# yunjinli/visual-slam

Hardware: AMD Instinct MI355X
Metric: stereo frames/sec, detect+describe (1500 feats) + stereo match, 752x480 (higher is better)
Workload: dtype u8/f32/f64; 1 GPU; synthetic 752x480 stereo, 1500 feats/frame (BASELINE configs[1]); independent streams per GPU (configs[3]); inputs_resident_in_hbm=True, distinct_stereo_pairs_per_gpu=1024, distinct_scenes_per_gpu=64, stereo_frames_per_pass_per_gpu=1024, hip_streams=2, stereo_frames_per_launch=512, num_features=1500, match=threshold 70, ratio 1.2, cross-check

## Files before the change

### visual-slam_amd/csrc/detect.hip

```cpp
#include <type_traits>

#include "vsl_common.h"

#ifndef K1_ROWS
#define K1_ROWS 60
#endif
#ifndef K1_ROWS_SMALL
#define K1_ROWS_SMALL 29
#endif
#define VSL_QUALITY_LEVEL 0.01
#define K1_WLIST 384
#define K1_COLS 60

__device__ __forceinline__ int reflect101(int i, int n) { return i < 0 ? -i : (i >= n ? 2 * n - 2 - i : i); }

struct RowF {
  float rx, ry;
};

struct RowRaw {
  unsigned l, m, r;
};

typedef __amdgpu_buffer_rsrc_t ImgSrd;
__device__ __forceinline__ RowRaw rowload(ImgSrd img, int w, int yr, unsigned xm, unsigned xe, unsigned xp) {
  const int row = yr * w;
  RowRaw o;
  o.l = __builtin_amdgcn_raw_buffer_load_b8(img, (int)xm, row, 0);
  o.m = __builtin_amdgcn_raw_buffer_load_b8(img, (int)xe, row, 0);
  o.r = __builtin_amdgcn_raw_buffer_load_b8(img, (int)xp, row, 0);
  return o;
}

__device__ __forceinline__ RowF rowfilt(RowRaw p, float s, float s2) {
  const float l = (float)p.l, m = (float)p.m, r = (float)p.r;
  RowF o;
  o.rx = r - l;
  float t = s * l;
  t = t + s2 * m;
  t = t + s * r;
  o.ry = t;
  return o;
}

__device__ __forceinline__ float from_lane_below(float v) {
  return __builtin_bit_cast(float, __builtin_amdgcn_update_dpp(0, __builtin_bit_cast(int, v), 0x138, 0xf, 0xf, true));
}
__device__ __forceinline__ float from_lane_above(float v) {
  return __builtin_bit_cast(float, __builtin_amdgcn_update_dpp(0, __builtin_bit_cast(int, v), 0x130, 0xf, 0xf, true));
}

__device__ __forceinline__ double dpp_below_f64(double v) {
  const uint64_t b = __builtin_bit_cast(uint64_t, v);
  const uint32_t lo = (uint32_t)__builtin_amdgcn_update_dpp(0, (int)(uint32_t)b, 0x138, 0xf, 0xf, true);
  const uint32_t hi = (uint32_t)__builtin_amdgcn_update_dpp(0, (int)(uint32_t)(b >> 32), 0x138, 0xf, 0xf, true);
  return __builtin_bit_cast(double, ((uint64_t)hi << 32) | lo);
}

__device__ __forceinline__ double dpp_above_f64(double v) {
  const uint64_t b = __builtin_bit_cast(uint64_t, v);
  const uint32_t lo = (uint32_t)__builtin_amdgcn_update_dpp(0, (int)(uint32_t)b, 0x130, 0xf, 0xf, true);
  const uint32_t hi = (uint32_t)__builtin_amdgcn_update_dpp(0, (int)(uint32_t)(b >> 32), 0x130, 0xf, 0xf, true);
  return __builtin_bit_cast(double, ((uint64_t)hi << 32) | lo);
}

__device__ __forceinline__ float fmax3(float a, float b, float c) {
  float r;
  asm("v_max3_f32 %0, %1, %2, %3" : "=v"(r) : "v"(a), "v"(b), "v"(c));
  return r;
}

__device__ __forceinline__ float fmax2(float a, float b) {
  float r;
  asm("v_max_f32 %0, %1, %2" : "=v"(r) : "v"(a), "v"(b));
  return r;
}

#define K1_SQRT_FLOOR 0x1p-100f
__device__ __forceinline__ float fast_sqrt_rn(float t) {
  const float y = __builtin_amdgcn_rsqf(__builtin_fmaxf(t, K1_SQRT_FLOOR));
  const float r = t * y;
  const float e = __builtin_fmaf(-r, r, t);
  return __builtin_fmaf(e, 0.5f * y, r);
}
__device__ __forceinline__ float sqrt_rn(float t) {
  float r = fast_sqrt_rn(t);
  const bool small = t < K1_SQRT_FLOOR;
  if (__builtin_amdgcn_ballot_w64(small) != 0ull) {
    asm volatile("" ::: "memory");
    const bool rare = small && t > 0.f;
    if (__builtin_amdgcn_ballot_w64(rare) != 0ull) {
      asm volatile("" ::: "memory");
      if (rare) r = sqrtf(t);
    }
  }
  return r;
}

__global__ void sqrt_check_kernel(uint32_t lo, uint32_t hi, unsigned long long* bad) {
  const uint64_t stride = (uint64_t)gridDim.x * blockDim.x;
  unsigned long long n = 0;
  for (uint64_t b = (uint64_t)lo + blockIdx.x * blockDim.x + threadIdx.x; b <= hi; b += stride) {
    const float t = __builtin_bit_cast(float, (uint32_t)b);
    n += __builtin_bit_cast(uint32_t, fast_sqrt_rn(t)) != __builtin_bit_cast(uint32_t, sqrtf(t));
  }
  if (n) atomicAdd(bad, n);
}

__global__ void detect_init_kernel(int32_t* meta, int first, int n) {
  const int i = blockIdx.x * blockDim.x + threadIdx.x;
  if (i < n) {
    meta[(size_t)(first + i) * VSL_META_STRIDE + VSL_META_MAX] = INT32_MIN;
    meta[(size_t)(first + i) * VSL_META_STRIDE + VSL_META_NCAND] = 0;
  }
}

template <bool STORE_RESPONSE, int ROWS>
__global__ __launch_bounds__(256) void min_eig_response_kernel(const uint8_t* __restrict__ images,
                                                               float* __restrict__ response, int32_t* __restrict__ meta,
                                                               uint64_t* __restrict__ cand, size_t cand_cap, int w, int h,
                                                               int first, int wlist_cap, int n_images, int tiles_x, int tiles_y) {
  __shared__ uint64_t list[4][K1_WLIST];
  __shared__ int wave_n[4], wave_max[4], g_base;
  __shared__ double xbuf[4][2][66];
  const int tiles = tiles_x * tiles_y;
  int img_i, tile;
  if (n_images >= 8) {
    const int xcd = blockIdx.x & 7, sl = blockIdx.x >> 3;
    img_i = (sl / tiles) * 8 + xcd;
    tile = sl - (sl / tiles) * tiles;
  } else {
    img_i = blockIdx.x / tiles;
    tile = blockIdx.x - img_i * tiles;
  }
  if (img_i >= n_images) return;
  const int bx = tile % tiles_x, by = tile / tiles_x;
  const int slot = first + img_i;
  const ImgSrd img = __builtin_amdgcn_make_buffer_rsrc((void*)(images + (size_t)slot * w * h), 0, w * h, 0x00020000);
  float* __restrict__ resp = response + (size_t)slot * w * h;
  const int lane = threadIdx.x & 63;
  const int wave = __builtin_amdgcn_readfirstlane(threadIdx.x >> 6);
  const int xs = bx * K1_COLS;
  const int y0 = (by * 4 + wave) * ROWS;
  int n_wave = 0;
  int own_max = INT32_MIN;
  if (y0 < h) {
    const float s = (float)(1.0 / (4.0 * 3.0 * 255.0));
    const float s2 = 2.0f * s;
    const int x = xs - 2 + lane;
    const unsigned xe = (unsigned)reflect101(min(max(x, -1), w), w);
    const unsigned xm = (unsigned)reflect101((int)xe - 1, w), xp = (unsigned)reflect101((int)xe + 1, w);
    const bool own_col = lane >= 2 && lane < 2 + K1_COLS && x < w;
    const bool cand_col = own_col && x >= 1 && x < w - 1;
    const unsigned long long cand_lanes = __builtin_amdgcn_ballot_w64(cand_col);

    struct R3 {
      double xx, xy, yy;
    };
    R3 ra = {0, 0, 0}, rb = ra, bs = ra;
    float va = 0.f, vb = 0.f, hA = 0.f, hB = 0.f, hC = 0.f;
    RowF fA = {0.f, 0.f}, fB = fA, fC = fA;
    int prev_ye = -100, pre_row = -100;
    RowRaw pre = {0u, 0u, 0u};
    float vmax = -3.0e38f;
    const int y_end = min(h, y0 + ROWS);
    auto step = [&](auto steady_tag, auto even_tag, int q, R3& r2, R3& r1, float& v_mid_slot, float& v_dn_slot, float& h_up,
                    float& h_mid, float& h_dn, RowF& f0, RowF& f1, RowF& f2) {
      constexpr bool STEADY = decltype(steady_tag)::value;
      constexpr bool EVEN = decltype(even_tag)::value;
      if (STEADY) {
        f2 = rowfilt(pre, s, s2);
        pre = rowload(img, w, min(q + 2, h - 1), xm, xe, xp);
      } else {
        const int ye = reflect101(min(max(q, -1), h), h);
        if (ye == prev_ye + 1 && ye + 1 < h) {
          if (pre_row != ye + 1) pre = rowload(img, w, ye + 1, xm, xe, xp);
          f2 = rowfilt(pre, s, s2);
        } else {
          f0 = rowfilt(rowload(img, w, reflect101(ye - 1, h), xm, xe, xp), s, s2);
          f1 = rowfilt(rowload(img, w, ye, xm, xe, xp), s, s2);
          f2 = rowfilt(rowload(img, w, reflect101(ye + 1, h), xm, xe, xp), s, s2);
        }
        pre_row = min(ye + 2, h - 1);
        pre = rowload(img, w, pre_row, xm, xe, xp);
        prev_ye = ye;
      }
      const float dx = (f0.rx + f2.rx) * s + f1.rx * s2;
      const float dy = f2.ry - f0.ry;
      const double dxx = (double)(dx * dx), dxy = (double)(dx * dy), dyy = (double)(dy * dy);
      R3 cur;
      {
        xbuf[wave][0][lane + 1] = dxx;
        xbuf[wave][1][lane + 1] = dxy;
        asm volatile("" ::: "memory");
        const double lxx = xbuf[wave][0][lane], uxx = xbuf[wave][0][lane + 2];
        const double lxy = xbuf[wave][1][lane], uxy = xbuf[wave][1][lane + 2];
        asm volatile("" ::: "memory");
        cur.xx = (lxx + dxx) + uxx;
        cur.xy = (lxy + dxy) + uxy;
        cur.yy = (dpp_below_f64(dyy) + dyy) + dpp_above_f64(dyy);
      }
      const int y = q - 1;
      double Axx, Axy, Ayy;
      if (EVEN) {
        bs.xx = r1.xx + cur.xx;
        bs.xy = r1.xy + cur.xy;
        bs.yy = r1.yy + cur.yy;
        Axx = r2.xx + bs.xx;
        Axy = r2.xy + bs.xy;
        Ayy = r2.yy + bs.yy;
      } else {
        Axx = bs.xx + cur.xx;
        Axy = bs.xy + cur.xy;
        Ayy = bs.yy + cur.yy;
      }
      r2 = cur;
      const float X = (float)Axx, b = (float)Axy, Y = (float)Ayy;
      const float xpy = X + Y, d = 0.5f * (X - Y);
      float t = d * d;
      t = t + b * b;
      const float v_dn = __builtin_fmaf(0.5f, xpy, -sqrt_rn(t));
      float h_tmp;
      asm volatile("s_nop 1\n\tv_max_f32_dpp %0, %2, %2 wave_shr:1 row_mask:0xf bank_mask:0xf bound_ctrl:0\n\t"
                   "v_max_f32_dpp %1, %2, %0 wave_shl:1 row_mask:0xf bank_mask:0xf bound_ctrl:0"
                   : "=&v"(h_tmp), "=&v"(h_dn)
                   : "v"(v_dn));
      if (own_col && y >= y0 && y < y_end) {
        if (STORE_RESPONSE) resp[y * w + x] = v_dn;
        vmax = fmax2(vmax, v_dn);
      }
      const float v_mid = v_mid_slot;
      const int yc = q - 2;
      if (yc >= y0 && yc < y_end && yc >= 1 && yc < h - 1) {
        const float m9 = fmax3(h_up, h_mid, h_dn);
        const bool ge0 = v_mid >= m9;
        if ((__builtin_amdgcn_ballot_w64(ge0) & cand_lanes) != 0ull) {
          const bool ge = ge0 && v_mid > 0.f;
          const unsigned long long mask = __builtin_amdgcn_ballot_w64(ge) & cand_lanes;
          if (cand_col && ge) {
            const uint32_t ob = (uint32_t)vsl_float_to_ordered(v_mid) ^ 0x80000000u;
            const uint64_t key = ((uint64_t)ob << 32) | ((uint32_t)yc << 16) | (uint32_t)x;
            const int p = n_wave + (int)__builtin_amdgcn_mbcnt_hi((uint32_t)(mask >> 32),
                                                                  __builtin_amdgcn_mbcnt_lo((uint32_t)mask, 0u));
            if (__builtin_expect(p < wlist_cap, 1)) {
              list[wave][p] = key;
            } else {
              const int g = atomicAdd(&meta[(size_t)slot * VSL_META_STRIDE + VSL_META_NCAND], 1);
              if ((size_t)g < cand_cap) cand[(size_t)slot * cand_cap + g] = key;
            }
          }
          n_wave += __popcll(mask);
        }
      }
      v_dn_slot = v_dn;
    };
    const int q_first = y0 - 2, q_last = y_end + 1;
    typedef std::integral_constant<bool, true> Steady;
    typedef std::integral_constant<bool, false> Generic;
    typedef std::integral_constant<bool, true> Even;
    typedef std::integral_constant<bool, false> Odd;
#define K1_STEP_E0(T, q) step(T{}, Even{}, q, ra, rb, va, vb, hA, hB, hC, fA, fB, fC)
#define K1_STEP_O1(T, q) step(T{}, Odd{}, q, rb, ra, vb, va, hB, hC, hA, fB, fC, fA)
#define K1_STEP_E2(T, q) step(T{}, Even{}, q, ra, rb, va, vb, hC, hA, hB, fC, fA, fB)
#define K1_STEP_O3(T, q) step(T{}, Odd{}, q, rb, ra, vb, va, hA, hB, hC, fA, fB, fC)
#define K1_STEP_E4(T, q) step(T{}, Even{}, q, ra, rb, va, vb, hB, hC, hA, fB, fC, fA)
#define K1_STEP_O5(T, q) step(T{}, Odd{}, q, rb, ra, vb, va, hC, hA, hB, fC, fA, fB)
    constexpr int K1_OPEN = (ROWS + 4) % 6;
    static_assert(K1_OPEN == 3 || K1_OPEN == 4, "opening sequence written for 3 or 4 steps");
#define K1_STRIP(T)                                \
  K1_STEP_E0(Generic, q_first);                    \
  K1_STEP_O1(T, q_first + 1);                      \
  K1_STEP_E2(T, q_first + 2);                      \
  if constexpr (K1_OPEN == 3) {                    \
    for (int q = q_first + 3; q <= q_last; q += 6) { \
      K1_STEP_O3(T, q);                            \
      K1_STEP_E4(T, q + 1);                        \
      K1_STEP_O5(T, q + 2);                        \
      K1_STEP_E0(T, q + 3);                        \
      K1_STEP_O1(T, q + 4);                        \
      K1_STEP_E2(T, q + 5);                        \
    }                                              \
  } else {                                         \
    K1_STEP_O3(T, q_first + 3);                    \
    for (int q = q_first + 4; q <= q_last; q += 6) { \
      K1_STEP_E4(T, q);                            \
      K1_STEP_O5(T, q + 1);                        \
      K1_STEP_E0(T, q + 2);                        \
      K1_STEP_O1(T, q + 3);                        \
      K1_STEP_E2(T, q + 4);                        \
      K1_STEP_O3(T, q + 5);                        \
    }                                              \
  }
    if (q_first >= 1 && q_last + 1 < h) {
      K1_STRIP(Steady)
    } else {
      K1_STRIP(Generic)
    }
#undef K1_STRIP
#undef K1_STEP_E0
#undef K1_STEP_O1
#undef K1_STEP_E2
#undef K1_STEP_O3
#undef K1_STEP_E4
#undef K1_STEP_O5
#pragma unroll
    for (int o = 32; o > 0; o >>= 1) vmax = fmaxf(vmax, __shfl_xor(vmax, o));
    own_max = vsl_float_to_ordered(vmax);
    if (lane == 0) atomicMax(&meta[(size_t)slot * VSL_META_STRIDE + VSL_META_MAX], own_max);
  }
  if (lane == 0) wave_max[wave] = own_max;
  __syncthreads();
  int kept = min(n_wave, wlist_cap);
  {
    const float wg_max = vsl_ordered_to_float(max(max(wave_max[0], wave_max[1]), max(wave_max[2], wave_max[3])));
    if (wg_max > 0.f && kept > 0) {
      const float thr = (float)((double)wg_max * VSL_QUALITY_LEVEL);
      const uint32_t floor_hi = (uint32_t)vsl_float_to_ordered(thr) ^ 0x80000000u;
      const int have = kept;
      kept = 0;
      for (int i0 = 0; i0 < have; i0 += 64) {
        const int i = i0 + lane;
        const uint64_t key = i < have ? list[wave][i] : 0ull;
        const bool keep = i < have && (uint32_t)(key >> 32) > floor_hi;
        const unsigned long long m = __builtin_amdgcn_ballot_w64(keep);
        if (keep) list[wave][kept + (int)__builtin_amdgcn_mbcnt_hi((uint32_t)(m >> 32), __builtin_amdgcn_mbcnt_lo((uint32_t)m, 0u))] = key;
        kept += __popcll(m);
      }
    }
  }
  if (lane == 0) wave_n[wave] = kept;
  __syncthreads();
  const int c0 = wave_n[0], c1 = wave_n[1], c2 = wave_n[2], c3 = wave_n[3];
  const int n = c0 + c1 + c2 + c3;
  if (n == 0) return;
  if (threadIdx.x == 0) g_base = atomicAdd(&meta[(size_t)slot * VSL_META_STRIDE + VSL_META_NCAND], n);
  __syncthreads();
  const int base = g_base + (wave > 0 ? c0 : 0) + (wave > 1 ? c1 : 0) + (wave > 2 ? c2 : 0);
  const int mine = wave_n[wave];
  for (int i = lane; i < mine; i += 64)
    if ((size_t)(base + i) < cand_cap) cand[(size_t)slot * cand_cap + base + i] = list[wave][i];
}

#define SEL_THREADS 1024
#define SEL_CHUNK 8192
#define SEL_BINS 1024
#define SEL_MAX_BLOCKERS 6
static_assert(SEL_THREADS <= 1024 && SEL_MAX_BLOCKERS * 10 <= 64, "blocker packing");

struct SelShared {
  int wave_tot[16];
  int hist[256];
  unsigned long long sel_prefix;
  int sel_k;
  int n_chunk;
};

__device__ __forceinline__ int block_scan(bool p, int* wave_tot, int& total) {
  const int lane = threadIdx.x & 63, wave = __builtin_amdgcn_readfirstlane(threadIdx.x >> 6);
  const unsigned long long m = __ballot(p);
  const int within = (int)__builtin_amdgcn_mbcnt_hi((uint32_t)(m >> 32), __builtin_amdgcn_mbcnt_lo((uint32_t)m, 0u));
  const int mine = __popcll(m);
  __syncthreads();
  if (lane == 0) wave_tot[wave] = mine;
  __syncthreads();
  int x = wave_tot[lane & 15];
  x += __builtin_amdgcn_update_dpp(0, x, 0x111, 0xf, 0xf, true);
  x += __builtin_amdgcn_update_dpp(0, x, 0x112, 0xf, 0xf, true);
  x += __builtin_amdgcn_update_dpp(0, x, 0x114, 0xf, 0xf, true);
  x += __builtin_amdgcn_update_dpp(0, x, 0x118, 0xf, 0xf, true);
  total = __builtin_amdgcn_readlane(x, 15);
  return __builtin_amdgcn_readlane(x, wave) - mine + within;
}

#define SEL_MAX_CELLS 6144
#define SEL_ACC_VALID 0x40u
#define SEL_HEAD_EMPTY 0xFFFFu
#define SEL_KEYS_PADDED (SEL_CHUNK + SEL_CHUNK / 32)
#define SEL_PHYS(i) ((i) + ((i) >> 5))
#define SEL_GRID_BYTES (SEL_MAX_CELLS * 2 * 2)
#define SEL_STAGE_PAD (SEL_CHUNK * 4 - SEL_THREADS * 4 - SEL_GRID_BYTES)
#define SEL_LDS_BYTES (SEL_KEYS_PADDED * 8 + 2048 + SEL_THREADS * 4 * 3 + SEL_GRID_BYTES + SEL_STAGE_PAD)
static_assert(SEL_STAGE_PAD >= 0, "ranking staging array");
static_assert(SEL_LDS_BYTES <= 160 * 1024 - 39344, "selection kernel LDS budget: one describe_tile_kernel workgroup fits beside it");

__device__ __forceinline__ uint32_t sel_xchg16(volatile uint16_t* arr, int idx, uint32_t v) {
  uint32_t* word = (uint32_t*)arr + (idx >> 1);
  const int s = (idx & 1) * 16;
  uint32_t old = *(volatile uint32_t*)word;
  for (;;) {
    const uint32_t got = atomicCAS(word, old, (old & ~(0xFFFFu << s)) | (v << s));
    if (got == old) break;
    old = got;
  }
  return (old >> s) & 0xFFFFu;
}

__device__ __forceinline__ int sel_head_rank(uint32_t h) { return h == SEL_HEAD_EMPTY ? -1 : (int)h; }

__device__ __forceinline__ void sel_acc_insert(volatile uint16_t* arr, int idx, uint32_t b) {
  uint32_t* word = (uint32_t*)arr + (idx >> 1);
  const int s = (idx & 1) * 16;
  uint32_t old = *(volatile uint32_t*)word;
  for (;;) {
    const uint32_t cur = (old >> s) & 0xFFFFu;
    if ((cur & 0xFF00u) != 0u) break;
    const uint32_t got = atomicCAS(word, old, old | (b << (s + ((cur & 0xFFu) ? 8 : 0))));
    if (got == old) break;
    old = got;
  }
}

template <int LOGK, int REPS>
__device__ __forceinline__ void sel_sort_blocked(uint64_t* keys, int tid0, int log_n) {
  constexpr int KPT = 1 << LOGK;
  for (int m = 1; m <= log_n; m++) {
    const int k = 1 << m;
    for (int top = m - 1; top >= 0;) {
      const int b = top >= LOGK - 1 ? top - (LOGK - 1) : 0;
      const int nb = top - b + 1;
#pragma unroll 1
      for (int tid = tid0; tid < REPS * SEL_THREADS; tid += SEL_THREADS) {
      const int t_hi = tid >> b, t_lo = tid & ((1 << b) - 1);
      const int i0 = (t_hi << (b + LOGK)) | t_lo;
      uint64_t rk[KPT];
#pragma unroll
      for (int r = 0; r < KPT; r++) rk[r] = keys[SEL_PHYS(i0 | (r << b))];
#pragma unroll
      for (int x = LOGK - 1; x >= 0; x--) {
        if (x < nb) {
#pragma unroll
          for (int r = 0; r < KPT; r++) {
            if ((r & (1 << x)) == 0) {
              const bool desc = ((i0 | (r << b)) & k) == 0;
              const uint64_t u = rk[r], v = rk[r | (1 << x)];
              const bool sw = desc ? (u < v) : (u > v);
              rk[r] = sw ? v : u;
              rk[r | (1 << x)] = sw ? u : v;
            }
          }
        }
      }
#pragma unroll
      for (int r = 0; r < KPT; r++) keys[SEL_PHYS(i0 | (r << b))] = rk[r];
      }
      __syncthreads();
      top = b - 1;
    }
  }
}

template <bool GRID_GLOBAL>
__global__ __launch_bounds__(SEL_THREADS) void select_kernel(const uint64_t* __restrict__ cand_all,
                                                             int32_t* meta,
                                                             int32_t* __restrict__ kp_xy, int32_t* __restrict__ kp_count,
                                                             int w, int h, size_t cand_cap, int F, int first,
                                                             int num_features, int border, double quality,
                                                             uint32_t* __restrict__ grid_scratch, int bucket_cap) {
  __shared__ __align__(16) unsigned char smem[SEL_LDS_BYTES];
  const int slot = first + blockIdx.x;
  const uint64_t* __restrict__ cand = cand_all + (size_t)slot * cand_cap;
  const int n_cand_raw = meta[(size_t)slot * VSL_META_STRIDE + VSL_META_NCAND];
  const int n_cand = min(n_cand_raw, (int)cand_cap);
  const int gw = (w + 7) / 8 + 2, gh = (h + 7) / 8 + 2, cells = (gw * gh + 1) & ~1;
  uint64_t* keys = (uint64_t*)smem;
  uint32_t* keys32 = (uint32_t*)smem;
  SelShared* sh = (SelShared*)(smem + SEL_KEYS_PADDED * 8);
  int* next = (int*)(smem + SEL_KEYS_PADDED * 8 + 2048);
  volatile uint16_t* acc = GRID_GLOBAL ? (volatile uint16_t*)(grid_scratch + (size_t)slot * cells) : (volatile uint16_t*)(next + 3 * SEL_THREADS);
  volatile uint16_t* head = acc + cells;
  unsigned long long* node = (unsigned long long*)next;
  int* state = next + 2 * SEL_THREADS;
  const int tid = threadIdx.x;

  int n_acc = 0, n_out = 0;
  unsigned long long hi = ~0ull;
  int32_t* out = kp_xy + (size_t)slot * F * 2;
  const float maxv = vsl_ordered_to_float(meta[(size_t)slot * VSL_META_STRIDE + VSL_META_MAX]);
  const float thr = (float)((double)maxv * quality);
  const unsigned long long floor_key =
      (((unsigned long long)((uint32_t)vsl_float_to_ordered(thr) ^ 0x80000000u)) << 32) | 0xFFFFFFFFull;
  int remaining = 0;
  int* bcount = next;
  int* bstart = next + SEL_THREADS;
  int* bcursor = next + 2 * SEL_THREADS;
  uint32_t* stage = (uint32_t*)bcursor;
  static_assert(SEL_BINS == SEL_THREADS, "one bin per thread");
  const uint32_t hi_max = (uint32_t)vsl_float_to_ordered(maxv) ^ 0x80000000u;
  const uint32_t hi_floor = (uint32_t)vsl_float_to_ordered(thr) ^ 0x80000000u;
  int bshift = 16;
  while (bshift < 31 && (hi_max >> bshift) - (hi_floor >> bshift) >= (uint32_t)SEL_BINS) bshift++;
  const uint32_t bin_top = hi_max >> bshift;
  bool bucket_sort = false;
  if (maxv > 0.f) {
    bcount[tid] = 0;
    if (tid == 0) sh->n_chunk = 0;
    __syncthreads();
    for (int i = tid; i < n_cand; i += SEL_THREADS) {
      const unsigned long long key = cand[i];
      if (key > floor_key) {
        const uint32_t kb = min((uint32_t)(key >> 32) >> bshift, bin_top);
        atomicAdd(&bcount[bin_top - kb], 1);
      }
    }
    __syncthreads();
    const int c = bcount[tid];
    int x = c;
    const int lane = tid & 63, wv = tid >> 6;
#pragma unroll
    for (int o = 1; o < 64; o <<= 1) {
      const int y = __shfl_up(x, o);
      if (lane >= o) x += y;
    }
    int cmax = c;
#pragma unroll
    for (int o = 32; o > 0; o >>= 1) cmax = max(cmax, __shfl_xor(cmax, o));
    if (lane == 63) sh->wave_tot[wv] = x;
    if (lane == 0) sh->hist[wv] = cmax;
    __syncthreads();
    int off = 0, fullest = 0;
    remaining = 0;
#pragma unroll
    for (int k = 0; k < 16; k++) {
      off += k < wv ? sh->wave_tot[k] : 0;
      remaining += sh->wave_tot[k];
      fullest = max(fullest, sh->hist[k]);
    }
    bstart[tid] = off + x - c;
    bcursor[tid] = 0;
    bucket_sort = remaining <= SEL_CHUNK && fullest <= bucket_cap;
    __syncthreads();
  }
  if (!bucket_sort) {
    for (int i = tid; i < cells; i += SEL_THREADS) ((volatile uint32_t*)acc)[i] = i < (cells >> 1) ? 0u : ~0u;
    __syncthreads();
  }
  bool compact = false;

  while (remaining > 0 && n_acc < num_features) {
    unsigned long long lo = 0;
    if (remaining > SEL_CHUNK) {
      unsigned long long prefix = 0;
      int k = SEL_CHUNK;
      for (int shift = 56; shift >= 0; shift -= 8) {
        for (int i = tid; i < 256; i += SEL_THREADS) sh->hist[i] = 0;
        __syncthreads();
        const unsigned long long pmask = shift == 56 ? 0ull : (~0ull << (shift + 8));
        for (int i = tid; i < n_cand; i += SEL_THREADS) {
          const unsigned long long key = cand[i];
          if (key < hi && key > floor_key && (key & pmask) == prefix) atomicAdd(&sh->hist[(int)((key >> shift) & 255)], 1);
        }
        __syncthreads();
        if (tid == 0) {
          int kk = k, d = 255;
          for (; d > 0; d--) {
            if (sh->hist[d] >= kk) break;
            kk -= sh->hist[d];
          }
          sh->sel_k = kk;
          sh->sel_prefix = prefix | ((unsigned long long)d << shift);
        }
        __syncthreads();
        k = sh->sel_k;
        prefix = sh->sel_prefix;
        __syncthreads();
      }
      lo = prefix;
    }
    int n_chunk;
    if (bucket_sort) {
      for (int i = tid; i < n_cand; i += SEL_THREADS) {
        const unsigned long long key = cand[i];
        if (key > floor_key) {
          const int bin = (int)(bin_top - min((uint32_t)(key >> 32) >> bshift, bin_top));
          const int p = bstart[bin] + atomicAdd(&bcursor[bin], 1);
          keys[SEL_PHYS(p)] = key;
        }
      }
      __syncthreads();
      n_chunk = remaining;
      for (int p = tid; p < n_chunk; p += SEL_THREADS) {
        const unsigned long long key = keys[SEL_PHYS(p)];
        const int bin = (int)(bin_top - min((uint32_t)(key >> 32) >> bshift, bin_top));
        const int s0 = bstart[bin], e0 = s0 + bcount[bin];
        int larger = 0;
        for (int q = s0; q < e0; q++) larger += keys[SEL_PHYS(q)] > key;
        stage[s0 + larger] = (uint32_t)key;
      }
      __syncthreads();
      for (int p = tid; p < n_chunk; p += SEL_THREADS) keys32[p] = stage[p];
      __syncthreads();
      for (int i = tid; i < cells; i += SEL_THREADS) ((volatile uint32_t*)acc)[i] = i < (cells >> 1) ? 0u : ~0u;
      __syncthreads();
      compact = true;
      bucket_sort = false;
    } else {
      if (tid == 0) sh->n_chunk = 0;
      __syncthreads();
      for (int i = tid; i < n_cand; i += SEL_THREADS) {
        const unsigned long long key = cand[i];
        if (key >= lo && key < hi && key > floor_key) {
          const int p = atomicAdd(&sh->n_chunk, 1);
          if (p < SEL_CHUNK) keys[SEL_PHYS(p)] = key;
        }
      }
      __syncthreads();
      n_chunk = min(sh->n_chunk, SEL_CHUNK);
      int N = 1024;
      while (N < n_chunk) N <<= 1;
      for (int i = n_chunk + tid; i < N; i += SEL_THREADS) keys[SEL_PHYS(i)] = 0ull;
      __syncthreads();
      if (N >= 2048) {
        if (N == 8192) sel_sort_blocked<2, 2>(keys, tid, 13);
        else if (N == 4096) sel_sort_blocked<2, 1>(keys, tid, 12);
        else sel_sort_blocked<1, 1>(keys, tid, 11);
      } else {
        for (int k = 2; k <= N; k <<= 1) {
          for (int j = k >> 1; j > 0; j >>= 1) {
            for (int t = tid; t < (N >> 1); t += SEL_THREADS) {
              const int i = ((t & ~(j - 1)) << 1) | (t & (j - 1));
              const int l = i | j;
              const uint64_t a = keys[SEL_PHYS(i)], b = keys[SEL_PHYS(l)];
              const bool desc = (i & k) == 0;
              if (desc ? (a < b) : (a > b)) {
                keys[SEL_PHYS(i)] = b;
                keys[SEL_PHYS(l)] = a;
              }
            }
            __syncthreads();
          }
        }
      }
    }
    for (int r0 = 0; r0 < n_chunk && n_acc < num_features; r0 += SEL_THREADS) {
      const int r = r0 + tid;
      int px = 0, py = 0, cell = 0;
      bool alive = false;
      if (r < n_chunk) {
        const uint32_t pix = compact ? keys32[r] : (uint32_t)(keys[SEL_PHYS(r)] & 0xFFFFFFFFull);
        py = (int)(pix >> 16);
        px = (int)(pix & 0xFFFFu);
        cell = ((py >> 3) + 1) * gw + (px >> 3) + 1;
        const int lx = px & 7, ly = py & 7;
        int near = 0;
#pragma unroll
        for (int oy = -1; oy <= 1; oy++) {
          const int row = cell + oy * gw;
          const uint32_t t0 = acc[row - 1], t1 = acc[row], t2 = acc[row + 1];
#pragma unroll
          for (int k = 0; k < 6; k++) {
            const uint32_t b = ((k >> 1) == 0 ? t0 : (k >> 1) == 1 ? t1 : t2) >> (8 * (k & 1));
            const int dx = lx - 8 * ((k >> 1) - 1) - (int)(b & 7u), dy = ly - 8 * oy - (int)((b >> 3) & 7u);
            const unsigned d2 = (unsigned)(dx * dx) + (unsigned)(dy * dy);
            near |= (int)((b & SEL_ACC_VALID) != 0u) & (int)(d2 < 64u);
          }
        }
        alive = near == 0;
      }
      state[tid] = alive ? 0 : 2;
      {
        const uint32_t prev = alive ? sel_xchg16(head, cell, (uint32_t)tid) : SEL_HEAD_EMPTY;
        const int nxt = sel_head_rank(prev);
        node[tid] = ((unsigned long long)(uint32_t)nxt << 32) | ((uint32_t)px | ((uint32_t)py << 16));
      }
      __syncthreads();
      int nb = 0;
      unsigned long long blk = 0ull;
      if (alive) {
#pragma unroll 1
        for (int oy = -1; oy <= 1; oy++) {
          const int row = cell + oy * gw;
          uint32_t h3[3];
#pragma unroll
          for (int k = 0; k < 3; k++) h3[k] = head[row + k - 1];
#pragma unroll
          for (int k = 0; k < 3; k++)
            for (int u = sel_head_rank(h3[k]); u >= 0;) {
              const unsigned long long nd = node[u];
              const int uu = u;
              u = (int)(nd >> 32);
              if (uu < tid) {
                const uint32_t q = (uint32_t)nd;
                const int dx = px - (int)(q & 0xFFFF), dy = py - (int)(q >> 16);
                if (dx * dx + dy * dy < 64) {
                  blk = (blk << 10) | (unsigned long long)(unsigned)uu;
                  nb++;
                }
              }
            }
        }
      }
      bool undecided = alive;
      while (__ballot(undecided) != 0ull) {
        if (undecided) {
          bool rej = false, blocked = false;
          if (nb <= SEL_MAX_BLOCKERS) {
#pragma unroll
            for (int k = 0; k < SEL_MAX_BLOCKERS; k++)
              if (k < nb) {
                const int su = ((volatile int*)state)[(int)(blk >> (10 * k)) & 1023];
                rej = rej || (su == 1);
                blocked = blocked || (su == 0);
              }
          } else {
            for (int k = 0; k < 9; k++)
                for (int u = sel_head_rank(head[cell + (k / 3 - 1) * gw + (k % 3 - 1)]), un = -1; u >= 0; u = un) {
                  const unsigned long long nd = node[u];
                  un = (int)(nd >> 32);
                  if (u < tid) {
                    const uint32_t q = (uint32_t)nd;
                    const int dx = px - (int)(q & 0xFFFF), dy = py - (int)(q >> 16);
                    if (dx * dx + dy * dy < 64) {
                      const int su = ((volatile int*)state)[u];
                      rej = rej || (su == 1);
                      blocked = blocked || (su == 0);
                    }
                  }
                }
          }
          const int ns = rej ? 2 : (blocked ? 0 : 1);
          if (ns) {
            ((volatile int*)state)[tid] = ns;
            undecided = false;
          }
        }
        __builtin_amdgcn_s_sleep(1);
      }
      __syncthreads();
      const bool accepted = alive && state[tid] == 1;
      int total = 0;
      const int rank = n_acc + block_scan(accepted, sh->wave_tot, total);
      const bool keep = accepted && rank < num_features;
      const bool inb = keep && px >= border && px < w - border && py >= border && py < h - border;
      int total_out = 0;
      const int pos = n_out + block_scan(inb, sh->wave_tot, total_out);
      if (inb) {
        out[2 * pos] = px;
        out[2 * pos + 1] = py;
      }
      if (keep) sel_acc_insert(acc, cell, SEL_ACC_VALID | (uint32_t)((py & 7) << 3) | (uint32_t)(px & 7));
      if (alive) head[cell] = (uint16_t)SEL_HEAD_EMPTY;
      n_acc = min(num_features, n_acc + total);
      n_out += total_out;
      __syncthreads();
    }
    hi = lo;
    remaining -= n_chunk;
  }
  if (tid == 0) {
    kp_count[slot] = n_out;
    meta[(size_t)slot * VSL_META_STRIDE + VSL_META_NCAND_LAST] = n_cand_raw;
    meta[(size_t)slot * VSL_META_STRIDE + VSL_META_MAX] = INT32_MIN;
    meta[(size_t)slot * VSL_META_STRIDE + VSL_META_NCAND] = 0;
  }
}

extern "C" int vsl_diag_sqrt_check(vsl_ctx* ctx, uint32_t lo_bits, uint32_t hi_bits, unsigned long long* n_mismatch) {
  if (!ctx || !n_mismatch || lo_bits > hi_bits || hi_bits > 0x7f7fffffu)
    return vsl_fail(ctx, VSL_ERR_INVALID, "vsl_diag_sqrt_check: bad range");
  VSL_HIP(ctx, hipSetDevice(ctx->device));
  void* d = nullptr;
  int rc = vsl_ctx_dscratch(ctx, sizeof(unsigned long long), &d);
  if (rc) return rc;
  VSL_HIP(ctx, hipMemsetAsync(d, 0, sizeof(unsigned long long), ctx->stream));
  hipLaunchKernelGGL(sqrt_check_kernel, dim3(4096), dim3(256), 0, ctx->stream, lo_bits, hi_bits, (unsigned long long*)d);
  VSL_CHECK_LAUNCH(ctx);
  VSL_HIP(ctx, hipMemcpyAsync(n_mismatch, d, sizeof(unsigned long long), hipMemcpyDeviceToHost, ctx->stream));
  VSL_HIP(ctx, hipStreamSynchronize(ctx->stream));
  return VSL_OK;
}

int vsl_launch_detect(vsl_ctx* ctx, vsl_frames* f, int first, int n, int num_features) {
  if (n <= 0) return VSL_OK;
  if (num_features < 1 || num_features > f->F)
    return vsl_fail(ctx, VSL_ERR_INVALID, "num_features %d not in [1, %d]", num_features, f->F);
  static_assert(sizeof(SelShared) <= 2048, "SelShared fits its LDS slot");
  const int cells = (((f->w + 7) / 8 + 2) * ((f->h + 7) / 8 + 2) + 1) & ~1;
  const bool grid_global = cells > SEL_MAX_CELLS;
  if (grid_global && !f->sel_grid) {
    VSL_HIP(ctx, hipMalloc((void**)&f->sel_grid, sizeof(uint32_t) * (size_t)cells * f->max_images));
  }
  const int w = f->w, h = f->h;
  {
    VslStage st(ctx, VSL_STAGE_RESPONSE);
    if (f->detect_meta_dirty)
      hipLaunchKernelGGL(detect_init_kernel, dim3((f->max_images + 255) / 256), dim3(256), 0, ctx->stream, f->meta, 0, f->max_images);
    f->detect_meta_dirty = true;
    const bool small = n < 8 && !f->store_response;
    const int rows = small ? K1_ROWS_SMALL : K1_ROWS;
    const int tiles_y = (h + 4 * rows - 1) / (4 * rows);
    const int tiles_x = (w + K1_COLS - 1) / K1_COLS;
    const dim3 k1_grid((unsigned)(tiles_x * tiles_y) * (unsigned)(n >= 8 ? 8 * ((n + 7) / 8) : n));
    const int wcap = ctx->k1_list_cap < 0 ? K1_WLIST : min(ctx->k1_list_cap, K1_WLIST);
    if (f->store_response)
      hipLaunchKernelGGL((min_eig_response_kernel<true, K1_ROWS>), k1_grid, dim3(256), 0, ctx->stream, f->images, f->response, f->meta,
                         f->cand, f->cand_cap, w, h, first, wcap, n, tiles_x, tiles_y);
    else if (small)
      hipLaunchKernelGGL((min_eig_response_kernel<false, K1_ROWS_SMALL>), k1_grid, dim3(256), 0, ctx->stream, f->images, f->response, f->meta,
                         f->cand, f->cand_cap, w, h, first, wcap, n, tiles_x, tiles_y);
    else
      hipLaunchKernelGGL((min_eig_response_kernel<false, K1_ROWS>), k1_grid, dim3(256), 0, ctx->stream, f->images, f->response, f->meta,
                         f->cand, f->cand_cap, w, h, first, wcap, n, tiles_x, tiles_y);
    VSL_CHECK_LAUNCH(ctx);
  }
  {
    VslStage st(ctx, VSL_STAGE_SELECT);
    if (grid_global)
      hipLaunchKernelGGL(select_kernel<true>, dim3(n), dim3(SEL_THREADS), 0, ctx->stream, f->cand, f->meta, f->kp_xy,
                         f->kp_count, w, h, f->cand_cap, f->F, first, num_features, 19, VSL_QUALITY_LEVEL, f->sel_grid, ctx->select_bucket_cap);
    else
      hipLaunchKernelGGL(select_kernel<false>, dim3(n), dim3(SEL_THREADS), 0, ctx->stream, f->cand, f->meta, f->kp_xy,
                         f->kp_count, w, h, f->cand_cap, f->F, first, num_features, 19, VSL_QUALITY_LEVEL, (uint32_t*)nullptr,
                         ctx->select_bucket_cap);
    VSL_CHECK_LAUNCH(ctx);
  }
  f->detect_meta_dirty = false;
  return VSL_OK;
}
```

Baseline: 382,300 frames/s.

## Keep selection candidates in registers, merge scans, drop barriers in NMS select

When the candidate count fits in one chunk, the select kernel now loads the candidates into registers once and reuses them for both the histogram and the bucket scatter, instead of reading global memory twice. Bucket ranking is hoisted out of the chunk loop and writes directly to an offset region, which removes a staging copy. The two block scans for accepted and in-border points are packed into one 16/16-bit scan, and volatile accesses become relaxed workgroup atomics with non-volatile LDS grid pointers, which removes a couple of barriers per chunk. The cost is higher register pressure, and the 16-bit packing assumes counts stay below 65536.

```diff
diff --git a/visual-slam_amd/csrc/detect.hip b/visual-slam_amd/csrc/detect.hip
--- a/visual-slam_amd/csrc/detect.hip
+++ b/visual-slam_amd/csrc/detect.hip
@@ -355,12 +355,12 @@
   int n_chunk;
 };
 
-__device__ __forceinline__ int block_scan(bool p, int* wave_tot, int& total) {
+__device__ __forceinline__ int block_scan(bool p, bool q, int* wave_tot, int& total) {
   const int lane = threadIdx.x & 63, wave = __builtin_amdgcn_readfirstlane(threadIdx.x >> 6);
-  const unsigned long long m = __ballot(p);
-  const int within = (int)__builtin_amdgcn_mbcnt_hi((uint32_t)(m >> 32), __builtin_amdgcn_mbcnt_lo((uint32_t)m, 0u));
-  const int mine = __popcll(m);
-  __syncthreads();
+  const unsigned long long m = __ballot(p), mq = __ballot(q);
+  const int within = (int)__builtin_amdgcn_mbcnt_hi((uint32_t)(m >> 32), __builtin_amdgcn_mbcnt_lo((uint32_t)m, 0u)) |
+                     (int)__builtin_amdgcn_mbcnt_hi((uint32_t)(mq >> 32), __builtin_amdgcn_mbcnt_lo((uint32_t)mq, 0u)) << 16;
+  const int mine = __popcll(m) | __popcll(mq) << 16;
   if (lane == 0) wave_tot[wave] = mine;
   __syncthreads();
   int x = wave_tot[lane & 15];
@@ -381,12 +381,23 @@
 #define SEL_STAGE_PAD (SEL_CHUNK * 4 - SEL_THREADS * 4 - SEL_GRID_BYTES)
 #define SEL_LDS_BYTES (SEL_KEYS_PADDED * 8 + 2048 + SEL_THREADS * 4 * 3 + SEL_GRID_BYTES + SEL_STAGE_PAD)
 static_assert(SEL_STAGE_PAD >= 0, "ranking staging array");
+#define SEL_KPT (SEL_CHUNK / SEL_THREADS)
+#define SEL_POS_UPPER (2 * SEL_PHYS(SEL_CHUNK / 2))
+static_assert(SEL_POS_UPPER + SEL_CHUNK / 2 <= 2 * SEL_KEYS_PADDED, "ranked positions behind the keys");
 static_assert(SEL_LDS_BYTES <= 160 * 1024 - 39344, "selection kernel LDS budget: one describe_tile_kernel workgroup fits beside it");
 
-__device__ __forceinline__ uint32_t sel_xchg16(volatile uint16_t* arr, int idx, uint32_t v) {
+template <bool GRID_GLOBAL> struct SelGrid {
+  typedef typename std::conditional<GRID_GLOBAL, volatile uint16_t, uint16_t>::type u16;
+  typedef typename std::conditional<GRID_GLOBAL, volatile uint32_t, uint32_t>::type u32;
+};
+
+template <class T16>
+__device__ __forceinline__ uint32_t sel_xchg16(T16* arr, int idx, uint32_t v) {
   uint32_t* word = (uint32_t*)arr + (idx >> 1);
   const int s = (idx & 1) * 16;
-  uint32_t old = *(volatile uint32_t*)word;
+  uint32_t old;
+  if constexpr (std::is_volatile<T16>::value) old = *(volatile uint32_t*)word;
+  else old = *word;
   for (;;) {
     const uint32_t got = atomicCAS(word, old, (old & ~(0xFFFFu << s)) | (v << s));
     if (got == old) break;
@@ -397,10 +408,13 @@
 
 __device__ __forceinline__ int sel_head_rank(uint32_t h) { return h == SEL_HEAD_EMPTY ? -1 : (int)h; }
 
-__device__ __forceinline__ void sel_acc_insert(volatile uint16_t* arr, int idx, uint32_t b) {
+template <class T16>
+__device__ __forceinline__ void sel_acc_insert(T16* arr, int idx, uint32_t b) {
   uint32_t* word = (uint32_t*)arr + (idx >> 1);
   const int s = (idx & 1) * 16;
-  uint32_t old = *(volatile uint32_t*)word;
+  uint32_t old;
+  if constexpr (std::is_volatile<T16>::value) old = *(volatile uint32_t*)word;
+  else old = *word;
   for (;;) {
     const uint32_t cur = (old >> s) & 0xFFFFu;
     if ((cur & 0xFF00u) != 0u) break;
@@ -466,8 +480,10 @@
   uint32_t* keys32 = (uint32_t*)smem;
   SelShared* sh = (SelShared*)(smem + SEL_KEYS_PADDED * 8);
   int* next = (int*)(smem + SEL_KEYS_PADDED * 8 + 2048);
-  volatile uint16_t* acc = GRID_GLOBAL ? (volatile uint16_t*)(grid_scratch + (size_t)slot * cells) : (volatile uint16_t*)(next + 3 * SEL_THREADS);
-  volatile uint16_t* head = acc + cells;
+  typedef typename SelGrid<GRID_GLOBAL>::u16 grid_u16;
+  typedef typename SelGrid<GRID_GLOBAL>::u32 grid_u32;
+  grid_u16* acc = GRID_GLOBAL ? (grid_u16*)(grid_scratch + (size_t)slot * cells) : (grid_u16*)(next + 3 * SEL_THREADS);
+  grid_u16* head = acc + cells;
   unsigned long long* node = (unsigned long long*)next;
   int* state = next + 2 * SEL_THREADS;
   const int tid = threadIdx.x;
@@ -491,15 +507,28 @@
   while (bshift < 31 && (hi_max >> bshift) - (hi_floor >> bshift) >= (uint32_t)SEL_BINS) bshift++;
   const uint32_t bin_top = hi_max >> bshift;
   bool bucket_sort = false;
+  const bool in_regs = n_cand <= SEL_CHUNK;
+  unsigned long long rk[SEL_KPT] = {};
   if (maxv > 0.f) {
     bcount[tid] = 0;
     if (tid == 0) sh->n_chunk = 0;
     __syncthreads();
-    for (int i = tid; i < n_cand; i += SEL_THREADS) {
-      const unsigned long long key = cand[i];
-      if (key > floor_key) {
-        const uint32_t kb = min((uint32_t)(key >> 32) >> bshift, bin_top);
-        atomicAdd(&bcount[bin_top - kb], 1);
+    if (in_regs) {
+#pragma unroll
+      for (int k = 0; k < SEL_KPT; k++) {
+        const int i = tid + k * SEL_THREADS;
+        rk[k] = i < n_cand ? cand[i] : 0ull;
+      }
+#pragma unroll
+      for (int k = 0; k < SEL_KPT; k++)
+        if (rk[k] > floor_key) atomicAdd(&bcount[bin_top - min((uint32_t)(rk[k] >> 32) >> bshift, bin_top)], 1);
+    } else {
+      for (int i = tid; i < n_cand; i += SEL_THREADS) {
+        const unsigned long long key = cand[i];
+        if (key > floor_key) {
+          const uint32_t kb = min((uint32_t)(key >> 32) >> bshift, bin_top);
+          atomicAdd(&bcount[bin_top - kb], 1);
+        }
       }
     }
     __syncthreads();
@@ -530,11 +559,71 @@
     bucket_sort = remaining <= SEL_CHUNK && fullest <= bucket_cap;
     __syncthreads();
   }
-  if (!bucket_sort) {
-    for (int i = tid; i < cells; i += SEL_THREADS) ((volatile uint32_t*)acc)[i] = i < (cells >> 1) ? 0u : ~0u;
-    __syncthreads();
-  }
+  if (!bucket_sort || in_regs)
+    for (int i = tid; i < cells; i += SEL_THREADS) ((grid_u32*)acc)[i] = i < (cells >> 1) ? 0u : ~0u;
+  if (!bucket_sort) __syncthreads();
   bool compact = false;
+  int pos_off = 0;
+  if (bucket_sort && remaining > 0) {
+    if (in_regs) {
+#pragma unroll
+      for (int k = 0; k < SEL_KPT; k++)
+        if (rk[k] > floor_key) {
+          const int bin = (int)(bin_top - min((uint32_t)(rk[k] >> 32) >> bshift, bin_top));
+          const int p = bstart[bin] + atomicAdd(&bcursor[bin], 1);
+          keys[SEL_PHYS(p)] = rk[k];
+        }
+      __syncthreads();
+      const bool upper = remaining <= SEL_CHUNK / 2;
+#pragma unroll
+      for (int k = 0; k < SEL_KPT; k++) {
+        const int p = tid + k * SEL_THREADS;
+        rk[k] = ~0ull;
+        if (p < remaining) {
+          const unsigned long long key = keys[SEL_PHYS(p)];
+          const int bin = (int)(bin_top - min((uint32_t)(key >> 32) >> bshift, bin_top));
+          const int s0 = bstart[bin], e0 = s0 + bcount[bin];
+          int larger = 0;
+          for (int q = s0; q < e0; q++) larger += keys[SEL_PHYS(q)] > key;
+          if (upper) keys32[SEL_POS_UPPER + s0 + larger] = (uint32_t)key;
+          else rk[k] = ((unsigned long long)(uint32_t)(s0 + larger) << 32) | (uint32_t)key;
+        }
+      }
+      __syncthreads();
+      if (upper) {
+        pos_off = SEL_POS_UPPER;
+      } else {
+#pragma unroll
+        for (int k = 0; k < SEL_KPT; k++)
+          if ((uint32_t)(rk[k] >> 32) < (uint32_t)SEL_CHUNK) keys32[(uint32_t)(rk[k] >> 32)] = (uint32_t)rk[k];
+        __syncthreads();
+      }
+    } else {
+      for (int i = tid; i < n_cand; i += SEL_THREADS) {
+        const unsigned long long key = cand[i];
+        if (key > floor_key) {
+          const int bin = (int)(bin_top - min((uint32_t)(key >> 32) >> bshift, bin_top));
+          const int p = bstart[bin] + atomicAdd(&bcursor[bin], 1);
+          keys[SEL_PHYS(p)] = key;
+        }
+      }
+      __syncthreads();
+      for (int p = tid; p < remaining; p += SEL_THREADS) {
+        const unsigned long long key = keys[SEL_PHYS(p)];
+        const int bin = (int)(bin_top - min((uint32_t)(key >> 32) >> bshift, bin_top));
+        const int s0 = bstart[bin], e0 = s0 + bcount[bin];
+        int larger = 0;
+        for (int q = s0; q < e0; q++) larger += keys[SEL_PHYS(q)] > key;
+        stage[s0 + larger] = (uint32_t)key;
+      }
+      __syncthreads();
+      for (int p = tid; p < remaining; p += SEL_THREADS) keys32[p] = stage[p];
+      __syncthreads();
+      for (int i = tid; i < cells; i += SEL_THREADS) ((grid_u32*)acc)[i] = i < (cells >> 1) ? 0u : ~0u;
+      __syncthreads();
+    }
+    compact = true;
+  }
 
   while (remaining > 0 && n_acc < num_features) {
     unsigned long long lo = 0;
@@ -567,32 +656,8 @@
       lo = prefix;
     }
     int n_chunk;
-    if (bucket_sort) {
-      for (int i = tid; i < n_cand; i += SEL_THREADS) {
-        const unsigned long long key = cand[i];
-        if (key > floor_key) {
-          const int bin = (int)(bin_top - min((uint32_t)(key >> 32) >> bshift, bin_top));
-          const int p = bstart[bin] + atomicAdd(&bcursor[bin], 1);
-          keys[SEL_PHYS(p)] = key;
-        }
-      }
-      __syncthreads();
+    if (compact) {
       n_chunk = remaining;
-      for (int p = tid; p < n_chunk; p += SEL_THREADS) {
-        const unsigned long long key = keys[SEL_PHYS(p)];
-        const int bin = (int)(bin_top - min((uint32_t)(key >> 32) >> bshift, bin_top));
-        const int s0 = bstart[bin], e0 = s0 + bcount[bin];
-        int larger = 0;
-        for (int q = s0; q < e0; q++) larger += keys[SEL_PHYS(q)] > key;
-        stage[s0 + larger] = (uint32_t)key;
-      }
-      __syncthreads();
-      for (int p = tid; p < n_chunk; p += SEL_THREADS) keys32[p] = stage[p];
-      __syncthreads();
-      for (int i = tid; i < cells; i += SEL_THREADS) ((volatile uint32_t*)acc)[i] = i < (cells >> 1) ? 0u : ~0u;
-      __syncthreads();
-      compact = true;
-      bucket_sort = false;
     } else {
       if (tid == 0) sh->n_chunk = 0;
       __syncthreads();
@@ -636,7 +701,7 @@
       int px = 0, py = 0, cell = 0;
       bool alive = false;
       if (r < n_chunk) {
-        const uint32_t pix = compact ? keys32[r] : (uint32_t)(keys[SEL_PHYS(r)] & 0xFFFFFFFFull);
+        const uint32_t pix = compact ? keys32[pos_off + r] :(uint32_t)(keys[SEL_PHYS(r)] & 0xFFFFFFFFull);
         py = (int)(pix >> 16);
         px = (int)(pix & 0xFFFFu);
         cell = ((py >> 3) + 1) * gw + (px >> 3) + 1;
@@ -689,7 +754,7 @@
             }
         }
       }
-      bool undecided = alive;
+      bool undecided = alive, accepted = false;
       while (__ballot(undecided) != 0ull) {
         if (undecided) {
           bool rej = false, blocked = false;
@@ -697,7 +762,7 @@
 #pragma unroll
             for (int k = 0; k < SEL_MAX_BLOCKERS; k++)
               if (k < nb) {
-                const int su = ((volatile int*)state)[(int)(blk >> (10 * k)) & 1023];
+                const int su = __hip_atomic_load(&state[(int)(blk >> (10 * k)) & 1023], __ATOMIC_RELAXED, __HIP_MEMORY_SCOPE_WORKGROUP);
                 rej = rej || (su == 1);
                 blocked = blocked || (su == 0);
               }
@@ -710,7 +775,7 @@
                     const uint32_t q = (uint32_t)nd;
                     const int dx = px - (int)(q & 0xFFFF), dy = py - (int)(q >> 16);
                     if (dx * dx + dy * dy < 64) {
-                      const int su = ((volatile int*)state)[u];
+                      const int su = __hip_atomic_load(&state[u], __ATOMIC_RELAXED, __HIP_MEMORY_SCOPE_WORKGROUP);
                       rej = rej || (su == 1);
                       blocked = blocked || (su == 0);
                     }
@@ -719,29 +784,31 @@
           }
           const int ns = rej ? 2 : (blocked ? 0 : 1);
           if (ns) {
-            ((volatile int*)state)[tid] = ns;
+            __hip_atomic_store(&state[tid], ns, __ATOMIC_RELAXED, __HIP_MEMORY_SCOPE_WORKGROUP);
             undecided = false;
+            accepted = ns == 1;
           }
         }
         __builtin_amdgcn_s_sleep(1);
       }
-      __syncthreads();
-      const bool accepted = alive && state[tid] == 1;
+      const bool inside = px >= border && px < w - border && py >= border && py < h - border;
       int total = 0;
-      const int rank = n_acc + block_scan(accepted, sh->wave_tot, total);
-      const bool keep = accepted && rank < num_features;
-      const bool inb = keep && px >= border && px < w - border && py >= border && py < h - border;
-      int total_out = 0;
-      const int pos = n_out + block_scan(inb, sh->wave_tot, total_out);
+      const int pre = block_scan(accepted, accepted && inside, sh->wave_tot, total);
+      const int lim = num_features - n_acc;
+      const bool cut = (total & 0xFFFF) > lim;
+      const bool keep = accepted && (pre & 0xFFFF) < lim;
+      const bool inb = keep && inside;
       if (inb) {
+        const int pos = n_out + (pre >> 16);
         out[2 * pos] = px;
         out[2 * pos + 1] = py;
       }
+      if (cut && accepted && (pre & 0xFFFF) == lim) sh->sel_k = pre >> 16;
       if (keep) sel_acc_insert(acc, cell, SEL_ACC_VALID | (uint32_t)((py & 7) << 3) | (uint32_t)(px & 7));
       if (alive) head[cell] = (uint16_t)SEL_HEAD_EMPTY;
-      n_acc = min(num_features, n_acc + total);
-      n_out += total_out;
-      __syncthreads();
+      n_acc = min(num_features, n_acc + (total & 0xFFFF));
+      __syncthreads();
+      n_out += cut ? sh->sel_k : total >> 16;
     }
     hi = lo;
     remaining -= n_chunk;
```

Measured after the change: 386,500 frames/s, median of 6. +1.1%, better.
